# aws/sagemaker-xgboost-container

Measured on NVIDIA H100. Metric: boosting rounds/sec, higher is better.
Workload: dtype int64

## Files before the change

sagemaker-xgboost-container_b200/csrc/engine.h:

```cpp
#pragma once
#include <cuda_runtime.h>
#include <cstdint>
#include <cstdio>
#include <stdexcept>
#include <string>
#include <vector>

namespace b200 {

struct Error : std::runtime_error { using std::runtime_error::runtime_error; };
#define B200_CHECK(cond, msg) do { if (!(cond)) throw ::b200::Error(std::string(msg)); } while (0)
#define CUDA_OK(expr) do { cudaError_t e_ = (expr); if (e_ != cudaSuccess) throw ::b200::Error( \
    std::string("CUDA error: ") + cudaGetErrorString(e_) + " at " + __FILE__ + ":" + std::to_string(__LINE__)); } while (0)

extern long long g_kernel_launches;

cudaStream_t engine_stream();
int engine_num_sms();

template <typename T> struct DevBuf {
  T* p = nullptr; size_t n = 0;
  DevBuf() = default;
  DevBuf(const DevBuf&) = delete; DevBuf& operator=(const DevBuf&) = delete;
  ~DevBuf() { release(); }
// ... 46 lines not shown
inline int objective_transform(int o) {
  if (o == kBinaryLogistic || o == kRegLogistic) return kTransformSigmoid;
  if (objective_is_log_link(o)) return kTransformExp;
  return o == kHinge ? kTransformHinge : kTransformNone;
}

struct TrainParam {
  int objective = kSquaredError;
  int num_class = 1;
  int max_depth = 6, max_leaves = 0, max_bin = 256;
  int lossguide = 0;
  float eta = 0.3f, lambda = 1.0f, alpha = 0.0f, gamma = 0.0f, min_child_weight = 1.0f, max_delta_step = 0.0f;
  float scale_pos_weight = 1.0f, subsample = 1.0f, colsample_bytree = 1.0f, colsample_bylevel = 1.0f, colsample_bynode = 1.0f;
  unsigned seed = 0;
  int num_parallel_tree = 1;
  float huber_slope = 1.0f, tweedie_variance_power = 1.5f, poisson_max_delta_step = 0.7f;
};

struct SplitCand {
  float loss_chg; int feature; int bin; int dleft; int ord;
  long long GL, HL;
};

struct TreeArrays {
  int *left, *right, *parent, *split_index, *split_bin;
  unsigned char* default_left;
  float *split_cond, *base_weight, *loss_chg, *sum_hess;
};

struct GrowState {
  unsigned* seg_begin; unsigned* seg_count;
  int* hist_slot;
  GH64* node_sum;
  float* root_gain; float* weight;
  SplitCand* best;
  SplitCand* best_group;
  int* level_nodes;
  int* level_count;
  int* build_nid; int* build_sub_nid; int* build_parent_slot; int* build_count;
  unsigned* build_prefix;
  int* part_action;
  unsigned* tile_prefix;
  unsigned long long* tile_desc;
  unsigned* part_ctl;
  int* n_nodes; int* n_leaves;
  int* depth; unsigned char* open; int* n_slots; int* lg_done;
  float* lower; float* upper;
  float* scales;
  unsigned* absmax;
};

}
```

sagemaker-xgboost-container_b200/csrc/grow.cu:

```cuda
#include "grow.h"
#include <algorithm>
#include <cmath>
#include <cstdlib>
#include <cstring>
#include "comm.h"

namespace b200 {

__global__ void pack_tree_kernel(TreeArrays t, const int* n_nodes, DevNode* out, int cap) {
  const int nn = *n_nodes;
  for (int i = blockIdx.x * blockDim.x + threadIdx.x; i < cap; i += gridDim.x * blockDim.x) {
    DevNode d;
    if (i < nn) { d.cond = t.split_cond[i]; d.left = t.left[i]; d.right = t.right[i]; d.fidx_dl = (unsigned)t.split_index[i] | ((unsigned)t.default_left[i] << 31); }
    else { d.cond = 0.f; d.left = -1; d.right = -1; d.fidx_dl = 0; }
    out[i] = d;
  }
}
__global__ void snapshot_h_kernel(const GH64* slot, long long* cache, size_t entries) {
  for (size_t e = (size_t)blockIdx.x * blockDim.x + threadIdx.x; e < entries; e += (size_t)gridDim.x * blockDim.x) cache[e] = slot[e].h;
}
__global__ void slot_from_cache_kernel(GH64* slot, const long long* cache, size_t entries) {
  for (size_t e = (size_t)blockIdx.x * blockDim.x + threadIdx.x; e < entries; e += (size_t)gridDim.x * blockDim.x) { GH64 v; v.g = 0; v.h = cache[e]; slot[e] = v; }
}
__global__ void gather_u32_kernel(const unsigned* src, const unsigned* idx, unsigned* dst, int64_t n) {
  const int64_t i = (int64_t)blockIdx.x * blockDim.x + threadIdx.x;
  if (i < n) dst[i] = src[idx[i]];
}

void* PinnedPool::take(size_t bytes) {
  bytes = (bytes + 255) & ~(size_t)255;
  while (cur < chunks.size() && off + bytes > chunks[cur].second) { ++cur; off = 0; }
  if (cur >= chunks.size()) { size_t sz = std::max<size_t>(bytes, 4u << 20); char* p = nullptr; CUDA_OK(cudaMallocHost(&p, sz)); chunks.emplace_back(p, sz); off = 0; }
  void* r = chunks[cur].first + off; off += bytes; return r;
}
static bool tail_by_position(const BinnedMatrix& bm) { return bm.tw == 4 && !bm.tail_in_gather; }

size_t TreeBuilder::carve(GrowState& gs, uintptr_t base) const {
  const size_t N = cap_nodes, L = max_level_nodes, nblocks = ngroups + (tw > 0 ? 1 : 0);
  size_t off = 0;
  auto take = [&](auto*& p, size_t bytes) { p = reinterpret_cast<std::remove_reference_t<decltype(p)>>(base + off); off += (bytes + 255) & ~(size_t)255; };
  take(gs.seg_begin, 4 * N); take(gs.seg_count, 4 * N); take(gs.hist_slot, 4 * N); take(gs.node_sum, 16 * N); take(gs.root_gain, 4 * N); take(gs.weight, 4 * N);
  take(gs.best, sizeof(SplitCand) * N); take(gs.best_group, sizeof(SplitCand) * N * nblocks);
  take(gs.level_nodes, 4 * (size_t)(kMaxDepth + 1) * L); take(gs.level_count, 4 * (kMaxDepth + 2));
  take(gs.build_nid, 4 * L); take(gs.build_sub_nid, 4 * L); take(gs.build_parent_slot, 4 * L); take(gs.build_count, 4); take(gs.build_prefix, 4 * (L + 1));
  take(gs.part_action, 4 * L); take(gs.tile_prefix, 4 * (L + 1));
  take(gs.tile_desc, 8 * ((size_t)max_tiles + 1)); gs.part_ctl = (unsigned*)(gs.tile_desc + max_tiles);
  take(gs.n_leaves, 4); take(gs.scales, 16); take(gs.absmax, 8);
  take(gs.depth, 4 * N); take(gs.open, N); take(gs.n_slots, 4); take(gs.lg_done, 4); take(gs.lower, 4 * N); take(gs.upper, 4 * N);
  return off;
}

void TreeBuilder::ensure(const BinnedMatrix& bm, int max_depth_, int K, int lg_iters_, int n_ic_) {
  const bool tail_pos_ = tail_by_position(bm);
  const int64_t stride_ = (bm.n + 63) & ~(int64_t)63;
  if (n == bm.n && F == bm.F && ngroups == bm.ngroups && tw == bm.tw && tail_pos == tail_pos_ && max_depth == max_depth_ && lg_iters == lg_iters_ &&
      n_ic == n_ic_ && gpair.n >= (size_t)stride_ * K + 512) return;
  if (lg_iters_ == 0) B200_CHECK(max_depth_ >= 1 && max_depth_ <= kMaxDepth, "max_depth must be in [1, 16] for the B200 depth-wise hist builder");
  n = bm.n; F = bm.F; ngroups = bm.ngroups; tw = bm.tw; tail_pos = tail_pos_; max_depth = max_depth_; lg_iters = lg_iters_; n_ic = n_ic_;
  gp_stride = stride_; root_h_valid = false;
  cudaStream_t s = engine_stream();
  if (peer_reduce_active()) {
    peer_reduce_close();
    DevBuf<unsigned> bar; bar.alloc(1); bar.zero(s);
    Comm::get().allreduce_max_u32(bar.p, 1, s);
    Comm::get().sync_stream(s);
  }
  for (auto& tg : graphs) tg.destroy();
  size_t pool_slots; int max_nodes;
// ... 3 lines not shown
  } else {
    max_nodes = (1 << (max_depth + 1)) - 1; max_level_nodes = 1 << (max_depth - 1); region = max_level_nodes;
    pool_slots = 2 * (size_t)region;
  }
  cap_nodes = (max_nodes + 15) & ~15;
  slot_stride = hist_slot_entries(ngroups, tw);
  const size_t pool_bytes = pool_slots * slot_stride * sizeof(GH64);
  size_t free_b = 0, total_b = 0; cudaMemGetInfo(&free_b, &total_b);
  B200_CHECK(pool_bytes < free_b / 2 + hist_pool.n * sizeof(GH64), "histogram pool for this max_depth / max_leaves / feature count does not fit in device memory");
  hist_pool.alloc(pool_slots * slot_stride);
  gpair.alloc((size_t)gp_stride * K + 512); gpair.zero(s); err.alloc(1); tree_index_dev.alloc(1);
  if (!leaf_scale.p) { leaf_scale.alloc(1); set_leaf_scale(1.0f); }
  root_h_cache.alloc(slot_stride);
  for (int i = 0; i < 2; ++i) { ridx[i].alloc(n); gp[i].alloc(n); tl[i].alloc(tail_pos ? n : 0); }
  max_tiles = (unsigned)((n + kPartTile - 1) / kPartTile) + max_level_nodes + 1;
  scratch.alloc(3 * (size_t)max_level_nodes + 8);
  state_block.alloc(carve(gs, 0)); state_block.zero(s);
  carve(gs, (uintptr_t)state_block.p);
  tree_block.alloc(tree_block_bytes(cap_nodes));
  const TreeBlock tb = tree_block_layout(tree_block.p, cap_nodes);
  gs.n_nodes = tb.n_nodes; ta = tb.t; packed.alloc(cap_nodes);
  ic_path.alloc(n_ic ? (size_t)cap_nodes * F : 0); ic_allowed.alloc(n_ic ? (size_t)cap_nodes * F : 0);
  ic_sets.alloc((size_t)n_ic * F); ic_sets_host.clear();
  hist_configure();
  global_n = n;
  if (Comm::get().distributed()) {
    peer_reduce_setup({{hist_pool.p, hist_pool.n * sizeof(GH64)}, {state_block.p, state_block.n}}, s);
    DevBuf<double> dsum; dsum.alloc(1); double v = (double)n;
    CUDA_OK(cudaMemcpyAsync(dsum.p, &v, sizeof v, cudaMemcpyHostToDevice, s));
    Comm::get().allreduce_sum_f64(dsum.p, 1, s);
    CUDA_OK(cudaMemcpyAsync(&v, dsum.p, sizeof v, cudaMemcpyDeviceToHost, s));
    Comm::get().sync_stream(s);
    global_n = (int64_t)v;
  }
}

void TreeBuilder::set_leaf_scale(float v) {
  cudaStream_t s = engine_stream();
  CUDA_OK(cudaMemcpyAsync(leaf_scale.p, &v, sizeof v, cudaMemcpyHostToDevice, s));
  Comm::get().sync_stream(s);
}

const unsigned char* TreeBuilder::upload_mask(const std::string& mask, int tree_index) {
  cudaStream_t s = engine_stream(); feat_mask.ensure(mask.size());
  CUDA_OK(cudaMemcpyAsync(feat_mask.p, mask.data(), mask.size(), cudaMemcpyHostToDevice, s));
  CUDA_OK(cudaMemcpyAsync(tree_index_dev.p, &tree_index, sizeof(int), cudaMemcpyHostToDevice, s));
  Comm::get().sync_stream(s); return feat_mask.p;
// ... 115 lines not shown
  for (int it = 0; it < in.lg_iters; ++it) {
    launch_apply_lossguide(apply_args(in, 0, 0, 0), it, s);
    const PartArgs pa = part_args(0, it == 0 ? kRootRows : 0, 1);
    timed(kProfPartition, [&] { launch_partition(pa, max_tiles, s); });
    launch_lg_copy_back(pa, ridx[0].p, gp[0].p, tl[0].p, max_tiles, s);
    launch_zero_build_slots(gs, hist_pool.p, slot_stride, 1, s);
    timed(kProfDeepHist, [&] { launch_hist_build(level_hist_args(0), num_sms, s); });
    if (dist) {
      launch_lg_stage(gs, hist_pool.p, slot_stride, 1, s);
      allreduce_hist(hist_pool.p + (size_t)kLgStageSlot * slot_stride, slot_stride * 2);
      launch_lg_stage(gs, hist_pool.p, slot_stride, 0, s);
    }
    launch_subtract(gs, hist_pool.p, slot_stride, 1, s);
    launch_eval(eval_args(in, 1, nullptr), 2, s);
  }
  for (int L = 0; L < D && in.lg_iters == 0; ++L) {
    const bool final_level = (L == D - 1);
    const int next_base = ((L + 1) & 1) * region, next_half = 1 << L;
    launch_apply(apply_args(in, L, next_base, next_half), s);
    if (final_level) break;
    PartArgs pa = part_args(L, L == 0 ? kRootRows : (L & 1) ^ 1, L & 1);
    pa.build_only = L == D - 2 ? 1 : 0;
    timed(kProfPartition, [&] { launch_partition(pa, max_tiles, s); });
    CUDA_OK(cudaMemsetAsync(hist_pool.p + (size_t)next_base * slot_stride, 0, (size_t)next_half * slot_stride * sizeof(GH64), s));
    timed(kProfDeepHist, [&] { launch_hist_build(level_hist_args(L & 1), num_sms, s); });
    allreduce_hist(hist_pool.p + (size_t)next_base * slot_stride, (size_t)next_half * slot_stride * 2);
    launch_subtract(gs, hist_pool.p, slot_stride, next_half, s);
    launch_eval(eval_args(in, L + 1, in.mask ? in.mask + (size_t)(L + 1) * bm.F : nullptr), 1 << (L + 1), s);
  }
  timed(kProfMargin, [&] { launch_update_margin(ta, gs.n_nodes, bm.bins_col, bm.n, bm.has_missing, in.margin, in.K, k, leaf_scale.p, s); });
  if (profile) prof_margin_rows += bm.n;
  pack_tree_kernel<<<(cap_nodes + 255) / 256, 256, 0, s>>>(ta, gs.n_nodes, packed.p, cap_nodes); ++g_kernel_launches;
  CUDA_OK(cudaGetLastError());
}
void TreeBuilder::end_segment() {
  cudaGraph_t graph = nullptr; cudaGraphExec_t exec = nullptr;
  CUDA_OK(cudaStreamEndCapture(engine_stream(), &graph));
  cudaError_t e = cudaGraphInstantiate(&exec, graph, 0);
  cudaGraphDestroy(graph);
  CUDA_OK(e);
  capturing->segs.push_back(exec);
}

void TreeBuilder::grow(const TreeInputs& in) {
  cudaStream_t s = engine_stream();
  static const bool no_graph = getenv("B200XGB_NO_GRAPH") != nullptr;
  if ((int)graphs.size() <= in.k) graphs.resize(in.k + 1);
// ... 159 lines not shown
```

sagemaker-xgboost-container_b200/csrc/tree.cu:

```cuda
#include <type_traits>
#include "engine.h"
#include "rng.h"
#include "tree.h"

namespace b200 {

__device__ __forceinline__ double threshold_l1(double w, double alpha) {
  if (w > +alpha) return w - alpha;
  if (w < -alpha) return w + alpha;
  return 0.0;
}
__device__ __forceinline__ float calc_weight(const TrainParamDev& p, double G, double H) {
  if (H < p.min_child_weight || H <= 0.0) return 0.0f;
  double dw = -threshold_l1(G, p.alpha) / (H + p.lambda);
  if (p.max_delta_step != 0.0f && fabs(dw) > p.max_delta_step) dw = copysign((double)p.max_delta_step, dw);
  return (float)dw;
}
__device__ __forceinline__ float gain_at_weight_f(float g, float h, float lambda, float w) {
  return -__fadd_rn(__fmul_rn(__fmul_rn(2.0f, g), w), __fmul_rn(__fmul_rn(__fadd_rn(h, lambda), w), w));
}
__device__ __forceinline__ float calc_gain_given_weight(const TrainParamDev& p, double G, double H, float w) {
  if (H <= 0.0) return 0.0f;
  if (p.max_delta_step == 0.0f) { double t = threshold_l1(G, p.alpha); return (float)(t * t / (H + p.lambda)); }
  return gain_at_weight_f((float)G, (float)H, p.lambda, w);
// ... 239 lines not shown
  const int cb = a.cut_ptrs[best.feature];
  const float thr = best.dleft ? (best.bin < 0 ? a.min_vals[best.feature] : a.cut_vals[cb + best.bin]) : a.cut_vals[cb + best.bin];
  t.left[nid] = Lc; t.right[nid] = Rc; t.split_index[nid] = best.feature; t.split_cond[nid] = thr;
  t.split_bin[nid] = best.bin; t.default_left[nid] = (unsigned char)best.dleft;
  t.base_weight[nid] = gs.weight[nid]; t.loss_chg[nid] = best.loss_chg; t.sum_hess[nid] = (float)((double)tot.h * ish);
  const int ch[2] = {Lc, Rc}; const float cw[2] = {wl, wr}; const double chh[2] = {HL, HR};
  for (int s = 0; s < 2; ++s) {
    const int c = ch[s];
    t.left[c] = -1; t.right[c] = -1; t.parent[c] = nid; t.split_index[c] = 0; t.split_bin[c] = -1; t.default_left[c] = 0;
    t.split_cond[c] = a.p.eta * cw[s]; t.base_weight[c] = a.p.eta * cw[s]; t.loss_chg[c] = 0.f; t.sum_hess[c] = (float)chh[s];
  }
  gs.node_sum[Lc].g = GLq; gs.node_sum[Lc].h = HLq; gs.node_sum[Rc].g = GRq; gs.node_sum[Rc].h = HRq;
  gs.seg_begin[Lc] = 0; gs.seg_count[Lc] = 0; gs.seg_begin[Rc] = 0; gs.seg_count[Rc] = 0;
}

__device__ __forceinline__ void plan_child_hists(const GrowState& gs, int r, int nid, const SplitCand& best, const GH64& tot, int Lc, int Rc,
                                                 int bld_slot, int sub_slot) {
  const bool fewer_right = tot.h - best.HL < best.HL;
  const int bld = fewer_right ? Rc : Lc, sub = fewer_right ? Lc : Rc;
  gs.hist_slot[bld] = bld_slot; gs.hist_slot[sub] = sub_slot;
  gs.build_nid[r] = bld; gs.build_sub_nid[r] = sub; gs.build_parent_slot[r] = gs.hist_slot[nid];
}

__global__ void __launch_bounds__(256) apply_kernel(ApplyArgs a) {
  __shared__ unsigned s_tmp[33];
  GrowState& gs = a.gs;
  const int L = a.level;
  const int cnt = gs.level_count[L];
  const int* nodes = gs.level_nodes + (size_t)L * a.max_level_nodes;
  unsigned* valid = a.scratch;
  unsigned* rank = a.scratch + a.max_level_nodes;
  unsigned* tiles = a.scratch + 2 * (size_t)a.max_level_nodes;
  const double isg = (double)gs.scales[2], ish = (double)gs.scales[3];
  if (L == 0 && threadIdx.x == 0 && cnt > 0) finish_root(a, ish);
  for (int i = threadIdx.x; i < cnt; i += blockDim.x) {
    const int nid = nodes[i];
    const SplitCand best = best_of_blocks(a, nid);
    valid[i] = split_is_valid(a.p, best, gs.node_sum[nid], L) ? 1u : 0u;
  }
  __syncthreads();
  if (a.p.max_leaves > 0 && threadIdx.x == 0) {
    int leaves = *gs.n_leaves;
    for (int i = 0; i < cnt; ++i) { if (valid[i]) { if (leaves >= a.p.max_leaves) valid[i] = 0; else ++leaves; } }
  }
  __syncthreads();
  const unsigned nvalid = block_exclusive_scan(valid, rank, cnt, s_tmp);
  const int n0 = *gs.n_nodes;
  const bool children_evaluated = (L + 1 < a.p.max_depth) || a.p.max_depth == 0;
  for (int i = threadIdx.x; i < cnt; i += blockDim.x) {
    const int nid = nodes[i];
    tiles[i] = (gs.seg_count[nid] + kPartTile - 1) / kPartTile;
    gs.part_action[i] = (int)valid[i];
    if (!valid[i]) continue;
    const SplitCand best = gs.best[nid];
    const GH64 tot = gs.node_sum[nid];
    const int r = (int)rank[i];
    const int Lc = n0 + 2 * r, Rc = Lc + 1;
    expand_node(a, nid, best, tot, Lc, Rc, isg, ish);
    if (children_evaluated) {
      int* nxt = gs.level_nodes + (size_t)(L + 1) * a.max_level_nodes;
      nxt[2 * r] = Lc; nxt[2 * r + 1] = Rc;
      plan_child_hists(gs, r, nid, best, tot, Lc, Rc, a.next_base + r, a.next_base + a.next_half + r);
    }
  }
  __syncthreads();
  const unsigned total_tiles = block_exclusive_scan(tiles, gs.tile_prefix, cnt, s_tmp);
  if (threadIdx.x == 0) {
    gs.tile_prefix[cnt] = total_tiles;
    *gs.n_nodes = n0 + 2 * (int)nvalid;
    *gs.n_leaves += (int)nvalid;
    gs.level_count[L + 1] = children_evaluated ? 2 * (int)nvalid : 0;
    *gs.build_count = children_evaluated ? (int)nvalid : 0;
  }
}

__global__ void __launch_bounds__(256) apply_lossguide_kernel(ApplyArgs a, int iter) {
  __shared__ unsigned long long s_key[8];
  GrowState& gs = a.gs;
  const double isg = (double)gs.scales[2], ish = (double)gs.scales[3];
  const int src = iter == 0 ? 0 : 1;
  const int cnt = gs.level_count[src];
  const int* nodes = gs.level_nodes + (size_t)src * a.max_level_nodes;
  if (iter == 0 && threadIdx.x == 0 && cnt > 0) finish_root(a, ish);
  for (int i = threadIdx.x; i < cnt; i += blockDim.x) {
    const int nid = nodes[i];
    gs.open[nid] = best_of_blocks(a, nid).loss_chg > 1e-6f ? 1 : 0;
  }
  __syncthreads();
  const int n0 = *gs.n_nodes;
  unsigned long long key = 0ull;
  for (int nid = threadIdx.x; nid < n0; nid += blockDim.x)
    if (gs.open[nid]) { unsigned long long k = ((unsigned long long)__float_as_uint(gs.best[nid].loss_chg) << 32) | (unsigned long long)(0xffffffffu - (unsigned)nid); key = k > key ? k : key; }
#pragma unroll
  for (int o = 16; o > 0; o >>= 1) { unsigned long long x = __shfl_xor_sync(0xffffffffu, key, o); key = x > key ? x : key; }
  if ((threadIdx.x & 31) == 0) s_key[threadIdx.x >> 5] = key;
  __syncthreads();
  if (threadIdx.x != 0) return;
  for (int w = 1; w < 8; ++w) key = s_key[w] > key ? s_key[w] : key;
  bool stop = *gs.lg_done != 0 || key == 0ull;
  int nid = 0; SplitCand best{}; GH64 tot{};
  if (!stop) {
    nid = (int)(0xffffffffu - (unsigned)(key & 0xffffffffull));
    best = gs.best[nid]; tot = gs.node_sum[nid];
    stop = !split_is_valid(a.p, best, tot, gs.depth[nid]) || (a.p.max_leaves > 0 && *gs.n_leaves == a.p.max_leaves);
  }
  if (stop) {
    *gs.lg_done = 1;
    gs.level_count[0] = 0; gs.level_count[1] = 0; *gs.build_count = 0; gs.part_action[0] = 0; gs.tile_prefix[0] = 0; gs.tile_prefix[1] = 0;
    return;
  }
  gs.open[nid] = 0;
  const int Lc = n0, Rc = n0 + 1, d = gs.depth[nid];
  expand_node(a, nid, best, tot, Lc, Rc, isg, ish);
  gs.depth[Lc] = d + 1; gs.depth[Rc] = d + 1; gs.open[Lc] = 0; gs.open[Rc] = 0;
  *gs.n_nodes = n0 + 2;
  const int leaves = *gs.n_leaves + 1;
  *gs.n_leaves = leaves;
  const bool children_evaluated = !(a.p.max_depth > 0 && d + 1 >= a.p.max_depth) && !(a.p.max_leaves > 0 && leaves >= a.p.max_leaves);
  gs.level_nodes[0] = nid; gs.level_count[0] = 1;
  gs.part_action[0] = children_evaluated ? 1 : 0;
  gs.tile_prefix[0] = 0; gs.tile_prefix[1] = children_evaluated ? (gs.seg_count[nid] + kPartTile - 1) / kPartTile : 0u;
  if (children_evaluated) {
    int* nxt = gs.level_nodes + (size_t)a.max_level_nodes;
    nxt[0] = Lc; nxt[1] = Rc; gs.level_count[1] = 2;
    const int slot = (*gs.n_slots)++;
    plan_child_hists(gs, 0, nid, best, tot, Lc, Rc, slot, gs.hist_slot[nid]);
    *gs.build_count = 1;
  } else { gs.level_count[1] = 0; *gs.build_count = 0; }
}

template <typename Pay>
__global__ void __launch_bounds__(256) lg_copy_back_kernel(PartArgs a, unsigned* ridx_dst, Pay* gp_dst, unsigned* tl_dst) {
  const GrowState& gs = a.gs;
  if (gs.level_count[0] <= 0 || !gs.part_action[0]) return;
  const int nid = gs.level_nodes[0];
  const unsigned b = gs.seg_begin[nid], c = gs.seg_count[nid];
  const Pay* gp_src = static_cast<const Pay*>(a.gp_next);
  for (unsigned p = b + blockIdx.x * blockDim.x + threadIdx.x; p < b + c; p += gridDim.x * blockDim.x) {
    ridx_dst[p] = a.ridx_next[p]; gp_dst[p] = gp_src[p];
    if (a.tl_next) tl_dst[p] = a.tl_next[p];
  }
}

__global__ void __launch_bounds__(256) zero_build_slots_kernel(GrowState gs, GH64* pool, size_t stride) {
  const int r = blockIdx.x;
  if (r >= *gs.build_count) return;
  GH64* h = pool + (size_t)gs.hist_slot[gs.build_nid[r]] * stride;
  GH64 z; z.g = 0; z.h = 0;
  for (size_t e = (size_t)blockIdx.y * blockDim.x + threadIdx.x; e < stride; e += (size_t)gridDim.y * blockDim.x) h[e] = z;
}

__global__ void __launch_bounds__(256) lg_stage_kernel(GrowState gs, GH64* pool, size_t stride, int to_stage) {
  if (*gs.build_count <= 0) return;
  GH64* slot = pool + (size_t)gs.hist_slot[gs.build_nid[0]] * stride;
  GH64* stage = pool + (size_t)kLgStageSlot * stride;
  for (size_t e = (size_t)blockIdx.x * blockDim.x + threadIdx.x; e < stride; e += (size_t)gridDim.x * blockDim.x) {
    if (to_stage) stage[e] = slot[e]; else slot[e] = stage[e];
  }
}

__device__ __forceinline__ int find_node_of_tile(const unsigned* tile_prefix, int cnt, unsigned tile) {
  int lo = 0, hi = cnt;
  while (hi - lo > 1) { int mid = (lo + hi) >> 1; if (tile_prefix[mid] <= tile) lo = mid; else hi = mid; }
  return lo;
}

constexpr unsigned long long kDescAggregate = 1ull << 62;
constexpr unsigned long long kDescPrefix = 2ull << 62;

__device__ __forceinline__ unsigned long long ld_relaxed_u64(const unsigned long long* p) {
  unsigned long long v; asm volatile("ld.relaxed.gpu.global.u64 %0, [%1];" : "=l"(v) : "l"(p) : "memory"); return v;
}
__device__ __forceinline__ void st_relaxed_u64(unsigned long long* p, unsigned long long v) {
  asm volatile("st.relaxed.gpu.global.u64 [%0], %1;" :: "l"(p), "l"(v) : "memory");
}

__device__ unsigned lookback_lefts(const unsigned long long* d, unsigned lt) {
  const int lane = threadIdx.x & 31;
  unsigned acc = 0;
  for (int hi = (int)lt - 1; hi >= 0; hi -= 32) {
    const int j = hi - lane;
    unsigned long long v = 0;
    if (j >= 0) { v = ld_relaxed_u64(d + j); while ((v >> 62) == 0) { __nanosleep(64); v = ld_relaxed_u64(d + j); } }
    const unsigned pref = __ballot_sync(0xffffffffu, (v >> 62) == 2);
    const int last = pref ? __ffs(pref) - 1 : 31;
    unsigned x = lane <= last ? (unsigned)v : 0u;
#pragma unroll
    for (int o = 16; o > 0; o >>= 1) x += __shfl_xor_sync(0xffffffffu, x, o);
    acc += x;
    if (pref) break;
  }
  return acc;
}

template <bool GONLY, bool TL>
__global__ void __launch_bounds__(256, GONLY ? (TL ? 5 : 6) : 4) part_kernel(PartArgs a) {
  typedef typename std::conditional<GONLY, float, float2>::type Pay;
  GrowState& gs = a.gs;
  __shared__ unsigned s_rid[kPartTile];
  __shared__ Pay s_gp[kPartTile];
  __shared__ unsigned s_tl[TL ? kPartTile : 1];
  __shared__ unsigned s_w[8];
  const int cnt = gs.level_count[a.level];
  const unsigned total = cnt > 0 ? gs.tile_prefix[cnt] : 0u;
  if (threadIdx.x == 0) s_w[0] = atomicAdd(gs.part_ctl, 1u);
  __syncthreads();
  const unsigned tile = s_w[0];
  __syncthreads();
  const int i = tile < total ? find_node_of_tile(gs.tile_prefix, cnt, tile) : 0;
  if (tile < total && gs.part_action[i]) {
    const int nid = gs.level_nodes[(size_t)a.level * a.max_level_nodes + i];
    const unsigned t0 = gs.tile_prefix[i], lt = tile - t0;
    const unsigned b = gs.seg_begin[nid], c = gs.seg_count[nid];
    const unsigned p0 = b + lt * kPartTile, p1 = (b + c < p0 + kPartTile) ? b + c : p0 + kPartTile;
    const unsigned nrows = p1 - p0;
    const int f = a.tree.split_index[nid];
    const int sb = a.tree.split_bin[nid], dl = a.tree.default_left[nid];
    const uint8_t* col = a.bins_col + (int64_t)f * a.n;
    const Pay* gp_cur = static_cast<const Pay*>(a.gp_cur);
    Pay* gp_next = static_cast<Pay*>(a.gp_next);
    const unsigned pt = p0 + threadIdx.x * 8;
    unsigned rows[8]; Pay gp[8]; unsigned tl[8]; unsigned char fl[8]; unsigned mine = 0;
#pragma unroll
    for (int j = 0; j < 8; ++j) {
      const unsigned p = pt + j;
      rows[j] = 0; gp[j] = Pay{}; tl[j] = 0u;
      if (p < p1) {
        rows[j] = a.ridx_cur ? a.ridx_cur[p] : p;
        if constexpr (GONLY) gp[j] = static_cast<const float*>(a.gp_cur)[(size_t)p * a.gp_cur_stride];
        else gp[j] = gp_cur[p];
        if constexpr (TL) tl[j] = a.tl_cur[p];
      }
    }
#pragma unroll
    for (int j = 0; j < 8; ++j) {
      if (pt + j < p1) {
        const int byte = col[rows[j]];
        const bool left = (a.has_missing && byte == kMissingBin) ? (dl != 0) : (byte <= sb);
        fl[j] = left ? 1 : 0; mine += fl[j];
      } else fl[j] = 2;
    }
    const int lane = threadIdx.x & 31, warp = threadIdx.x >> 5;
    unsigned x = mine;
#pragma unroll
    for (int o = 1; o < 32; o <<= 1) { unsigned y = __shfl_up_sync(0xffffffffu, x, o); if (lane >= o) x += y; }
    if (lane == 31) s_w[warp] = x;
    __syncthreads();
    unsigned woff = 0, tile_left = 0;
    for (int w = 0; w < 8; ++w) { if (w < warp) woff += s_w[w]; tile_left += s_w[w]; }
    unsigned long long* desc = gs.tile_desc + t0;
    if (threadIdx.x == 0) st_relaxed_u64(desc + lt, (lt == 0 ? kDescPrefix : kDescAggregate) | tile_left);
    unsigned lbefore = woff + x - mine;
#pragma unroll
    for (int j = 0; j < 8; ++j) {
      if (fl[j] == 2) continue;
      const unsigned jj = threadIdx.x * 8 + j;
      const unsigned slot = fl[j] ? lbefore++ : tile_left + (jj - lbefore);
      s_rid[slot] = rows[j]; s_gp[slot] = gp[j]; if constexpr (TL) s_tl[slot] = tl[j];
    }
    unsigned lefts_before = 0;
    if (warp == 0 && lt > 0) {
      lefts_before = lookback_lefts(desc, lt);
      if (lane == 0) st_relaxed_u64(desc + lt, kDescPrefix | (lefts_before + tile_left));
    }
    __syncthreads();
    if (threadIdx.x == 0) s_w[0] = lefts_before;
    __syncthreads();
    lefts_before = s_w[0];
    const unsigned rights_before = lt * kPartTile - lefts_before;
    const int Lc = a.tree.left[nid], Rc = a.tree.right[nid];
    bool write_left = true, write_right = true;
    if (a.build_only) { const bool build_right = gs.node_sum[Rc].h < gs.node_sum[Lc].h; write_left = !build_right; write_right = build_right; }
    const unsigned k0 = write_left ? 0u : tile_left, k1 = write_right ? nrows : tile_left;
    const unsigned dl0 = b + lefts_before, dr0 = b + c - 1 - rights_before + tile_left;
    for (unsigned k = k0 + threadIdx.x; k < k1; k += blockDim.x) {
      const unsigned dest = k < tile_left ? dl0 + k : dr0 - k;
      a.ridx_next[dest] = s_rid[k];
      gp_next[dest] = s_gp[k];
      if constexpr (TL) a.tl_next[dest] = s_tl[k];
    }
    if (threadIdx.x == 0) {
      if (lt == gs.tile_prefix[i + 1] - t0 - 1) {
        const unsigned nl = lefts_before + tile_left;
        gs.seg_begin[Lc] = b; gs.seg_count[Lc] = nl; gs.seg_begin[Rc] = b + nl; gs.seg_count[Rc] = c - nl;
      }
      if (a.rows_counter) { atomicAdd(a.rows_counter, (unsigned long long)nrows); atomicAdd(a.rows_counter + 1, (unsigned long long)(k1 - k0)); }
    }
  }
  __syncthreads();
  if (threadIdx.x == 0) { __threadfence(); s_w[0] = atomicAdd(gs.part_ctl + 1, 1u) == gridDim.x - 1 ? 1u : 0u; }
  __syncthreads();
  if (!s_w[0]) return;
  __threadfence();
  const int nb = *gs.build_count;
  for (int r = threadIdx.x; r < nb; r += blockDim.x) gs.build_prefix[r] = __ldcg(gs.seg_count + gs.build_nid[r]);
  __syncthreads();
  const unsigned tot = nb > 0 ? block_exclusive_scan(gs.build_prefix, gs.build_prefix, nb, s_rid ) : 0u;
  if (threadIdx.x == 0) gs.build_prefix[nb > 0 ? nb : 0] = tot;
}

struct PackedNode { unsigned feat; unsigned short bin_dl; unsigned short left; };
constexpr int kPackedNodesSmem = 2048;
static_assert(sizeof(PackedNode) == 8, "PackedNode is 8 B");

__global__ void __launch_bounds__(256) update_margin_kernel(TreeArrays t, const int* n_nodes, const uint8_t* bins_col, int64_t n, int has_missing,
                                                            float* margin, int K, int k, const float* leaf_scale) {
  __shared__ PackedNode s_nodes[kPackedNodesSmem];
  __shared__ float s_leaf[kPackedNodesSmem];
  const int nn = *n_nodes;
  const bool packed = nn <= kPackedNodesSmem && nn < 0xffff;
  if (packed) {
    for (int i = threadIdx.x; i < nn; i += blockDim.x) {
      PackedNode p; p.feat = (unsigned)t.split_index[i]; p.bin_dl = (unsigned short)((t.split_bin[i] + 1) | (t.default_left[i] ? 0x8000 : 0));
      const int l = t.left[i]; p.left = l < 0 ? 0xffff : (unsigned short)l;
      s_nodes[i] = p; s_leaf[i] = t.split_cond[i];
    }
    __syncthreads();
  }
  const int64_t base = (int64_t)blockIdx.x * 1024 + threadIdx.x;
  int nid[4]; bool done[4];
  const bool root_leaf = packed ? (s_nodes[0].left == 0xffff) : (t.left[0] == -1);
// ... 39 lines not shown
  GH64* hs = pool + (size_t)gs.hist_slot[sub] * stride;
  for (size_t e = (size_t)blockIdx.y * blockDim.x + threadIdx.x; e < stride; e += (size_t)gridDim.y * blockDim.x) {
    GH64 p = hp[e], b = hb[e]; GH64 o; o.g = p.g - b.g; o.h = p.h - b.h; hs[e] = o;
  }
}

void launch_init_tree(const GrowState& gs, const TreeArrays& t, unsigned n, cudaStream_t s) {
  init_tree_kernel<<<1, 32, 0, s>>>(gs, t, n); ++g_kernel_launches; CUDA_OK(cudaGetLastError());
}
void launch_scales(const GrowState& gs, int grad_bits, cudaStream_t s) { scales_kernel<<<1, 32, 0, s>>>(gs, grad_bits); ++g_kernel_launches; CUDA_OK(cudaGetLastError()); }
void launch_eval(const EvalArgs& a, int max_nodes_level, cudaStream_t s) {
  dim3 grid(max_nodes_level, a.ngroups + (a.tw > 0 ? 1 : 0)); eval_kernel<<<grid, 32 * kEvalSegs, 0, s>>>(a); ++g_kernel_launches; CUDA_OK(cudaGetLastError());
}
void launch_apply_lossguide(const ApplyArgs& a, int iter, cudaStream_t s) { apply_lossguide_kernel<<<1, 256, 0, s>>>(a, iter); ++g_kernel_launches; CUDA_OK(cudaGetLastError()); }
void launch_lg_copy_back(const PartArgs& a, unsigned* ridx_dst, void* gp_dst, unsigned* tl_dst, unsigned max_tiles, cudaStream_t s) {
  const unsigned grid = max_tiles < 1184u ? max_tiles : 1184u;
  if (a.g_only) lg_copy_back_kernel<float><<<grid, 256, 0, s>>>(a, ridx_dst, static_cast<float*>(gp_dst), tl_dst);
  else lg_copy_back_kernel<float2><<<grid, 256, 0, s>>>(a, ridx_dst, static_cast<float2*>(gp_dst), tl_dst);
  ++g_kernel_launches; CUDA_OK(cudaGetLastError());
}
void launch_zero_build_slots(const GrowState& gs, GH64* pool, size_t slot_entries, int max_build, cudaStream_t s) {
  dim3 grid(max_build, (unsigned)((slot_entries + 1023) / 1024)); zero_build_slots_kernel<<<grid, 256, 0, s>>>(gs, pool, slot_entries); ++g_kernel_launches; CUDA_OK(cudaGetLastError());
}
void launch_lg_stage(const GrowState& gs, GH64* pool, size_t slot_entries, int to_stage, cudaStream_t s) {
  lg_stage_kernel<<<(unsigned)((slot_entries + 1023) / 1024), 256, 0, s>>>(gs, pool, slot_entries, to_stage); ++g_kernel_launches; CUDA_OK(cudaGetLastError());
}
void launch_apply(const ApplyArgs& a, cudaStream_t s) { apply_kernel<<<1, 256, 0, s>>>(a); ++g_kernel_launches; CUDA_OK(cudaGetLastError()); }
void launch_partition(const PartArgs& a, unsigned max_tiles, cudaStream_t s) {
  CUDA_OK(cudaMemsetAsync(a.gs.tile_desc, 0, sizeof(unsigned long long) * ((size_t)max_tiles + 1), s));
  const bool tl = a.tl_cur != nullptr;
  if (a.g_only) { if (tl) part_kernel<true, true><<<max_tiles, 256, 0, s>>>(a); else part_kernel<true, false><<<max_tiles, 256, 0, s>>>(a); }
  else { if (tl) part_kernel<false, true><<<max_tiles, 256, 0, s>>>(a); else part_kernel<false, false><<<max_tiles, 256, 0, s>>>(a); }
  ++g_kernel_launches; CUDA_OK(cudaGetLastError());
}
void launch_update_margin(const TreeArrays& t, const int* n_nodes, const uint8_t* bins_col, int64_t n, int has_missing, float* margin, int K, int k,
                          const float* leaf_scale, cudaStream_t s) {
  if (n == 0) return;
  update_margin_kernel<<<(unsigned)((n + 1023) / 1024), 256, 0, s>>>(t, n_nodes, bins_col, n, has_missing, margin, K, k, leaf_scale); ++g_kernel_launches; CUDA_OK(cudaGetLastError());
}
void launch_subtract(const GrowState& gs, GH64* pool, size_t slot_entries, int max_build, cudaStream_t s) {
  dim3 grid(max_build, (unsigned)((slot_entries + 1023) / 1024)); subtract_kernel<<<grid, 256, 0, s>>>(gs, pool, slot_entries); ++g_kernel_launches; CUDA_OK(cudaGetLastError());
}

}
```

sagemaker-xgboost-container_b200/csrc/tree.h:

```cpp
#pragma once
#include "engine.h"

namespace b200 {

constexpr unsigned kPartTile = 2048;

struct TrainParamDev {
  float eta, lambda, alpha, gamma, min_child_weight, max_delta_step;
  int max_depth, max_leaves;
};

struct EvalArgs {
  const GH64* hist_pool; GrowState gs; const int* cut_ptrs; const unsigned char* feat_mask;
  TrainParamDev p; int F, ngroups, tw, ntail, has_missing, level, max_level_nodes;
  const int* monotone;
  const unsigned char* node_allowed;
  float colsample_bynode; unsigned seed; const int* tree_index;
};

struct ApplyArgs {
  GrowState gs; TreeArrays tree; const int* cut_ptrs; const float* cut_vals; const float* min_vals;
  TrainParamDev p; unsigned* scratch; int nblocks , level, max_level_nodes, next_base, next_half;
  const int* monotone;
  unsigned char* node_path; unsigned char* node_allowed; const unsigned char* ic_sets; int n_ic_sets, F;
// ... 22 lines not shown
  const float* gpos;
  const unsigned* ridx;
  const int* build_count;
  const int* build_nid;
  const unsigned* build_prefix;
  const unsigned* seg_begin;
  const int* hist_slot;
  const float* scales;
  GH64* hist_pool;
  GH64* node_sum;
  int ngroups;
  int ng_chunk;
  int accumulate_sum;
  int g_only;
  int window_rows;
  int force_gather;
  unsigned long long* rows_counter;
};

constexpr int kLgRootSlot = 0, kLgStageSlot = 1, kLgFirstFreeSlot = 2;
void launch_apply_lossguide(const ApplyArgs& a, int iter, cudaStream_t s);
void launch_lg_copy_back(const PartArgs& a, unsigned* ridx_dst, void* gp_dst, unsigned* tl_dst, unsigned max_tiles, cudaStream_t s);
void launch_zero_build_slots(const GrowState& gs, GH64* pool, size_t slot_entries, int max_build, cudaStream_t s);
void launch_lg_stage(const GrowState& gs, GH64* pool, size_t slot_entries, int to_stage, cudaStream_t s);
void launch_hist_build(const HistArgs& a, int num_sms, cudaStream_t stream);
void hist_configure();
const char* hist_last_kernel();
void launch_init_tree(const GrowState& gs, const TreeArrays& t, unsigned n, cudaStream_t s);
void launch_scales(const GrowState& gs, int grad_bits, cudaStream_t s);
void launch_eval(const EvalArgs& a, int max_nodes_level, cudaStream_t s);
void launch_apply(const ApplyArgs& a, cudaStream_t s);
void launch_partition(const PartArgs& a, unsigned max_tiles, cudaStream_t s);
void launch_update_margin(const TreeArrays& t, const int* n_nodes, const uint8_t* bins_col, int64_t n, int has_missing, float* margin, int K, int k,
                          const float* leaf_scale, cudaStream_t s);
void launch_subtract(const GrowState& gs, GH64* pool, size_t slot_entries, int max_build, cudaStream_t s);

}
```

Measured before the change: 74.99.

## Restructure partition kernel with precomputed node plans, cp.async payload staging, ballot compaction

Apply kernels now write a compact PartNode record (segment, tile offset, split feature/bin, children, flags) so each partition CTA loads one struct instead of chasing several tree arrays. Warp 0 finds the tile's node with a ballot search. Gradient and tail payloads are staged through cp.async into shared memory, and the compaction uses warp ballots with a source-index indirection. The last-block build_prefix scan is moved into new zero-slot kernels, which replace a memset. Occupancy bounds and the shared-memory carveout are raised, at the cost of added register and shared-memory pressure and more synchronization complexity.

Measured after the change: 76.82 (median of 6 runs). +2.4%, better.

```diff
diff --git a/sagemaker-xgboost-container_b200/csrc/engine.h b/sagemaker-xgboost-container_b200/csrc/engine.h
--- a/sagemaker-xgboost-container_b200/csrc/engine.h
+++ b/sagemaker-xgboost-container_b200/csrc/engine.h
@@ -92,6 +92,14 @@
   long long GL, HL;
 };
 
+struct PartNode {
+  unsigned seg_begin, seg_count;
+  unsigned tile0;
+  int feature, split_bin;
+  int left, right;
+  unsigned flags;
+};
+
 struct TreeArrays {
   int *left, *right, *parent, *split_index, *split_bin;
   unsigned char* default_left;
@@ -110,6 +118,7 @@
   int* build_nid; int* build_sub_nid; int* build_parent_slot; int* build_count;
   unsigned* build_prefix;
   int* part_action;
+  PartNode* part_node;
   unsigned* tile_prefix;
   unsigned long long* tile_desc;
   unsigned* part_ctl;
diff --git a/sagemaker-xgboost-container_b200/csrc/grow.cu b/sagemaker-xgboost-container_b200/csrc/grow.cu
--- a/sagemaker-xgboost-container_b200/csrc/grow.cu
+++ b/sagemaker-xgboost-container_b200/csrc/grow.cu
@@ -43,7 +43,7 @@
   take(gs.best, sizeof(SplitCand) * N); take(gs.best_group, sizeof(SplitCand) * N * nblocks);
   take(gs.level_nodes, 4 * (size_t)(kMaxDepth + 1) * L); take(gs.level_count, 4 * (kMaxDepth + 2));
   take(gs.build_nid, 4 * L); take(gs.build_sub_nid, 4 * L); take(gs.build_parent_slot, 4 * L); take(gs.build_count, 4); take(gs.build_prefix, 4 * (L + 1));
-  take(gs.part_action, 4 * L); take(gs.tile_prefix, 4 * (L + 1));
+  take(gs.part_action, 4 * L); take(gs.part_node, sizeof(PartNode) * L); take(gs.tile_prefix, 4 * (L + 1));
   take(gs.tile_desc, 8 * ((size_t)max_tiles + 1)); gs.part_ctl = (unsigned*)(gs.tile_desc + max_tiles);
   take(gs.n_leaves, 4); take(gs.scales, 16); take(gs.absmax, 8);
   take(gs.depth, 4 * N); take(gs.open, N); take(gs.n_slots, 4); take(gs.lg_done, 4); take(gs.lower, 4 * N); take(gs.upper, 4 * N);
@@ -93,7 +93,7 @@
   gs.n_nodes = tb.n_nodes; ta = tb.t; packed.alloc(cap_nodes);
   ic_path.alloc(n_ic ? (size_t)cap_nodes * F : 0); ic_allowed.alloc(n_ic ? (size_t)cap_nodes * F : 0);
   ic_sets.alloc((size_t)n_ic * F); ic_sets_host.clear();
-  hist_configure();
+  hist_configure(); part_configure();
   global_n = n;
   if (Comm::get().distributed()) {
     peer_reduce_setup({{hist_pool.p, hist_pool.n * sizeof(GH64)}, {state_block.p, state_block.n}}, s);
@@ -255,7 +255,7 @@
     PartArgs pa = part_args(L, L == 0 ? kRootRows : (L & 1) ^ 1, L & 1);
     pa.build_only = L == D - 2 ? 1 : 0;
     timed(kProfPartition, [&] { launch_partition(pa, max_tiles, s); });
-    CUDA_OK(cudaMemsetAsync(hist_pool.p + (size_t)next_base * slot_stride, 0, (size_t)next_half * slot_stride * sizeof(GH64), s));
+    launch_zero_level_slots(gs, hist_pool.p + (size_t)next_base * slot_stride, (size_t)next_half * slot_stride, s);
     timed(kProfDeepHist, [&] { launch_hist_build(level_hist_args(L & 1), num_sms, s); });
     allreduce_hist(hist_pool.p + (size_t)next_base * slot_stride, (size_t)next_half * slot_stride * 2);
     launch_subtract(gs, hist_pool.p, slot_stride, next_half, s);
diff --git a/sagemaker-xgboost-container_b200/csrc/tree.cu b/sagemaker-xgboost-container_b200/csrc/tree.cu
--- a/sagemaker-xgboost-container_b200/csrc/tree.cu
+++ b/sagemaker-xgboost-container_b200/csrc/tree.cu
@@ -1,3 +1,4 @@
+#include <algorithm>
 #include <type_traits>
 #include "engine.h"
 #include "rng.h"
@@ -285,6 +286,14 @@
   gs.build_nid[r] = bld; gs.build_sub_nid[r] = sub; gs.build_parent_slot[r] = gs.hist_slot[nid];
 }
 
+__device__ __forceinline__ void plan_partition(const GrowState& gs, int i, int nid, const SplitCand& best, const GH64& tot, int Lc, int Rc, unsigned tile0) {
+  PartNode pn;
+  pn.seg_begin = gs.seg_begin[nid]; pn.seg_count = gs.seg_count[nid]; pn.tile0 = tile0;
+  pn.feature = best.feature; pn.split_bin = best.bin; pn.left = Lc; pn.right = Rc;
+  pn.flags = (best.dleft ? 1u : 0u) | (tot.h - best.HL < best.HL ? 2u : 0u);
+  gs.part_node[i] = pn;
+}
+
 __global__ void __launch_bounds__(256) apply_kernel(ApplyArgs a) {
   __shared__ unsigned s_tmp[33];
   GrowState& gs = a.gs;
@@ -308,17 +317,20 @@
   }
   __syncthreads();
   const unsigned nvalid = block_exclusive_scan(valid, rank, cnt, s_tmp);
+  for (int i = threadIdx.x; i < cnt; i += blockDim.x) tiles[i] = valid[i] ? (gs.seg_count[nodes[i]] + kPartTile - 1) / kPartTile : 0u;
+  __syncthreads();
+  const unsigned total_tiles = block_exclusive_scan(tiles, gs.tile_prefix, cnt, s_tmp);
   const int n0 = *gs.n_nodes;
   const bool children_evaluated = (L + 1 < a.p.max_depth) || a.p.max_depth == 0;
   for (int i = threadIdx.x; i < cnt; i += blockDim.x) {
     const int nid = nodes[i];
-    tiles[i] = (gs.seg_count[nid] + kPartTile - 1) / kPartTile;
     gs.part_action[i] = (int)valid[i];
     if (!valid[i]) continue;
     const SplitCand best = gs.best[nid];
     const GH64 tot = gs.node_sum[nid];
     const int r = (int)rank[i];
     const int Lc = n0 + 2 * r, Rc = Lc + 1;
+    plan_partition(gs, i, nid, best, tot, Lc, Rc, gs.tile_prefix[i]);
     expand_node(a, nid, best, tot, Lc, Rc, isg, ish);
     if (children_evaluated) {
       int* nxt = gs.level_nodes + (size_t)(L + 1) * a.max_level_nodes;
@@ -327,7 +339,6 @@
     }
   }
   __syncthreads();
-  const unsigned total_tiles = block_exclusive_scan(tiles, gs.tile_prefix, cnt, s_tmp);
   if (threadIdx.x == 0) {
     gs.tile_prefix[cnt] = total_tiles;
     *gs.n_nodes = n0 + 2 * (int)nvalid;
@@ -374,6 +385,7 @@
   }
   gs.open[nid] = 0;
   const int Lc = n0, Rc = n0 + 1, d = gs.depth[nid];
+  plan_partition(gs, 0, nid, best, tot, Lc, Rc, 0u);
   expand_node(a, nid, best, tot, Lc, Rc, isg, ish);
   gs.depth[Lc] = d + 1; gs.depth[Rc] = d + 1; gs.open[Lc] = 0; gs.open[Rc] = 0;
   *gs.n_nodes = n0 + 2;
@@ -405,7 +417,24 @@
   }
 }
 
+__device__ void write_build_prefix(const GrowState& gs, unsigned* s_tmp ) {
+  const int nb = *gs.build_count;
+  for (int r = threadIdx.x; r < nb; r += blockDim.x) gs.build_prefix[r] = gs.seg_count[gs.build_nid[r]];
+  __syncthreads();
+  const unsigned tot = nb > 0 ? block_exclusive_scan(gs.build_prefix, gs.build_prefix, nb, s_tmp) : 0u;
+  if (threadIdx.x == 0) gs.build_prefix[nb > 0 ? nb : 0] = tot;
+}
+
+__global__ void __launch_bounds__(256) zero_level_slots_kernel(GrowState gs, GH64* slots, size_t entries) {
+  __shared__ unsigned s_tmp[33];
+  if (blockIdx.x == 0) write_build_prefix(gs, s_tmp);
+  GH64 z; z.g = 0; z.h = 0;
+  for (size_t e = (size_t)blockIdx.x * blockDim.x + threadIdx.x; e < entries; e += (size_t)gridDim.x * blockDim.x) slots[e] = z;
+}
+
 __global__ void __launch_bounds__(256) zero_build_slots_kernel(GrowState gs, GH64* pool, size_t stride) {
+  __shared__ unsigned s_tmp[33];
+  if (blockIdx.x == 0 && blockIdx.y == 0) write_build_prefix(gs, s_tmp);
   const int r = blockIdx.x;
   if (r >= *gs.build_count) return;
   GH64* h = pool + (size_t)gs.hist_slot[gs.build_nid[r]] * stride;
@@ -422,10 +451,19 @@
   }
 }
 
-__device__ __forceinline__ int find_node_of_tile(const unsigned* tile_prefix, int cnt, unsigned tile) {
-  int lo = 0, hi = cnt;
-  while (hi - lo > 1) { int mid = (lo + hi) >> 1; if (tile_prefix[mid] <= tile) lo = mid; else hi = mid; }
-  return lo;
+__device__ __forceinline__ int find_node_of_tile(const unsigned* tile_prefix, const int* level_count, unsigned tile) {
+  const int lane = threadIdx.x & 31;
+  const unsigned v0 = tile_prefix[lane];
+  const int cnt = *level_count;
+  int i = 0;
+  for (int base = 0; base <= cnt; base += 32) {
+    const int j = base + lane;
+    const unsigned v = base == 0 ? v0 : (j <= cnt ? tile_prefix[j] : 0xffffffffu);
+    const unsigned m = __ballot_sync(0xffffffffu, j <= cnt && v <= tile);
+    if (m) i = base + 31 - __clz(m);
+    if (m != 0xffffffffu) break;
+  }
+  return i < cnt ? i : -1;
 }
 
 constexpr unsigned long long kDescAggregate = 1ull << 62;
@@ -456,110 +494,122 @@
   return acc;
 }
 
+template <int B> __device__ __forceinline__ void cp_async(void* smem, const void* gmem) {
+  const unsigned s = (unsigned)__cvta_generic_to_shared(smem);
+  asm volatile("cp.async.ca.shared.global [%0], [%1], %2;" :: "r"(s), "l"(gmem), "n"(B) : "memory");
+}
+__device__ __forceinline__ void cp_async_wait_all() { asm volatile("cp.async.wait_all;" ::: "memory"); }
+
+template <bool GONLY, bool TL> constexpr int part_ctas_per_sm() { return GONLY ? (TL ? 7 : 8) : (TL ? 5 : 6); }
 template <bool GONLY, bool TL>
-__global__ void __launch_bounds__(256, GONLY ? (TL ? 5 : 6) : 4) part_kernel(PartArgs a) {
+__global__ void __launch_bounds__(256, part_ctas_per_sm<GONLY, TL>()) part_kernel(PartArgs a) {
   typedef typename std::conditional<GONLY, float, float2>::type Pay;
   GrowState& gs = a.gs;
   __shared__ unsigned s_rid[kPartTile];
+  __shared__ unsigned short s_src[kPartTile];
   __shared__ Pay s_gp[kPartTile];
   __shared__ unsigned s_tl[TL ? kPartTile : 1];
   __shared__ unsigned s_w[8];
-  const int cnt = gs.level_count[a.level];
-  const unsigned total = cnt > 0 ? gs.tile_prefix[cnt] : 0u;
-  if (threadIdx.x == 0) s_w[0] = atomicAdd(gs.part_ctl, 1u);
-  __syncthreads();
-  const unsigned tile = s_w[0];
-  __syncthreads();
-  const int i = tile < total ? find_node_of_tile(gs.tile_prefix, cnt, tile) : 0;
-  if (tile < total && gs.part_action[i]) {
-    const int nid = gs.level_nodes[(size_t)a.level * a.max_level_nodes + i];
-    const unsigned t0 = gs.tile_prefix[i], lt = tile - t0;
-    const unsigned b = gs.seg_begin[nid], c = gs.seg_count[nid];
-    const unsigned p0 = b + lt * kPartTile, p1 = (b + c < p0 + kPartTile) ? b + c : p0 + kPartTile;
-    const unsigned nrows = p1 - p0;
-    const int f = a.tree.split_index[nid];
-    const int sb = a.tree.split_bin[nid], dl = a.tree.default_left[nid];
-    const uint8_t* col = a.bins_col + (int64_t)f * a.n;
-    const Pay* gp_cur = static_cast<const Pay*>(a.gp_cur);
-    Pay* gp_next = static_cast<Pay*>(a.gp_next);
-    const unsigned pt = p0 + threadIdx.x * 8;
-    unsigned rows[8]; Pay gp[8]; unsigned tl[8]; unsigned char fl[8]; unsigned mine = 0;
-#pragma unroll
-    for (int j = 0; j < 8; ++j) {
-      const unsigned p = pt + j;
-      rows[j] = 0; gp[j] = Pay{}; tl[j] = 0u;
-      if (p < p1) {
-        rows[j] = a.ridx_cur ? a.ridx_cur[p] : p;
-        if constexpr (GONLY) gp[j] = static_cast<const float*>(a.gp_cur)[(size_t)p * a.gp_cur_stride];
-        else gp[j] = gp_cur[p];
-        if constexpr (TL) tl[j] = a.tl_cur[p];
-      }
-    }
-#pragma unroll
-    for (int j = 0; j < 8; ++j) {
-      if (pt + j < p1) {
-        const int byte = col[rows[j]];
-        const bool left = (a.has_missing && byte == kMissingBin) ? (dl != 0) : (byte <= sb);
-        fl[j] = left ? 1 : 0; mine += fl[j];
-      } else fl[j] = 2;
-    }
-    const int lane = threadIdx.x & 31, warp = threadIdx.x >> 5;
-    unsigned x = mine;
-#pragma unroll
-    for (int o = 1; o < 32; o <<= 1) { unsigned y = __shfl_up_sync(0xffffffffu, x, o); if (lane >= o) x += y; }
-    if (lane == 31) s_w[warp] = x;
-    __syncthreads();
-    unsigned woff = 0, tile_left = 0;
-    for (int w = 0; w < 8; ++w) { if (w < warp) woff += s_w[w]; tile_left += s_w[w]; }
-    unsigned long long* desc = gs.tile_desc + t0;
-    if (threadIdx.x == 0) st_relaxed_u64(desc + lt, (lt == 0 ? kDescPrefix : kDescAggregate) | tile_left);
-    unsigned lbefore = woff + x - mine;
-#pragma unroll
-    for (int j = 0; j < 8; ++j) {
-      if (fl[j] == 2) continue;
-      const unsigned jj = threadIdx.x * 8 + j;
-      const unsigned slot = fl[j] ? lbefore++ : tile_left + (jj - lbefore);
-      s_rid[slot] = rows[j]; s_gp[slot] = gp[j]; if constexpr (TL) s_tl[slot] = tl[j];
-    }
-    unsigned lefts_before = 0;
-    if (warp == 0 && lt > 0) {
-      lefts_before = lookback_lefts(desc, lt);
-      if (lane == 0) st_relaxed_u64(desc + lt, kDescPrefix | (lefts_before + tile_left));
-    }
-    __syncthreads();
-    if (threadIdx.x == 0) s_w[0] = lefts_before;
-    __syncthreads();
-    lefts_before = s_w[0];
-    const unsigned rights_before = lt * kPartTile - lefts_before;
-    const int Lc = a.tree.left[nid], Rc = a.tree.right[nid];
-    bool write_left = true, write_right = true;
-    if (a.build_only) { const bool build_right = gs.node_sum[Rc].h < gs.node_sum[Lc].h; write_left = !build_right; write_right = build_right; }
-    const unsigned k0 = write_left ? 0u : tile_left, k1 = write_right ? nrows : tile_left;
-    const unsigned dl0 = b + lefts_before, dr0 = b + c - 1 - rights_before + tile_left;
-    for (unsigned k = k0 + threadIdx.x; k < k1; k += blockDim.x) {
-      const unsigned dest = k < tile_left ? dl0 + k : dr0 - k;
-      a.ridx_next[dest] = s_rid[k];
-      gp_next[dest] = s_gp[k];
-      if constexpr (TL) a.tl_next[dest] = s_tl[k];
-    }
-    if (threadIdx.x == 0) {
-      if (lt == gs.tile_prefix[i + 1] - t0 - 1) {
-        const unsigned nl = lefts_before + tile_left;
-        gs.seg_begin[Lc] = b; gs.seg_count[Lc] = nl; gs.seg_begin[Rc] = b + nl; gs.seg_count[Rc] = c - nl;
-      }
-      if (a.rows_counter) { atomicAdd(a.rows_counter, (unsigned long long)nrows); atomicAdd(a.rows_counter + 1, (unsigned long long)(k1 - k0)); }
-    }
-  }
-  __syncthreads();
-  if (threadIdx.x == 0) { __threadfence(); s_w[0] = atomicAdd(gs.part_ctl + 1, 1u) == gridDim.x - 1 ? 1u : 0u; }
-  __syncthreads();
-  if (!s_w[0]) return;
-  __threadfence();
-  const int nb = *gs.build_count;
-  for (int r = threadIdx.x; r < nb; r += blockDim.x) gs.build_prefix[r] = __ldcg(gs.seg_count + gs.build_nid[r]);
-  __syncthreads();
-  const unsigned tot = nb > 0 ? block_exclusive_scan(gs.build_prefix, gs.build_prefix, nb, s_rid ) : 0u;
-  if (threadIdx.x == 0) gs.build_prefix[nb > 0 ? nb : 0] = tot;
+  __shared__ PartNode s_node;
+  __shared__ unsigned s_lt;
+  const int lane = threadIdx.x & 31, warp = threadIdx.x >> 5;
+  if (warp == 0) {
+    unsigned tile = 0;
+    if (lane == 0) tile = atomicAdd(gs.part_ctl, 1u);
+    tile = __shfl_sync(0xffffffffu, tile, 0);
+    const int i = find_node_of_tile(gs.tile_prefix, gs.level_count + a.level, tile);
+    unsigned w = 0;
+    if (i >= 0 && lane < 8) { w = reinterpret_cast<const unsigned*>(gs.part_node + i)[lane]; reinterpret_cast<unsigned*>(&s_node)[lane] = w; }
+    const unsigned t0 = __shfl_sync(0xffffffffu, w, 2);
+    if (lane == 0) s_lt = i >= 0 ? tile - t0 : ~0u;
+  }
+  __syncthreads();
+  const unsigned lt = s_lt;
+  if (lt == ~0u) return;
+  const unsigned p0 = s_node.seg_begin + lt * kPartTile, nrows = min(s_node.seg_begin + s_node.seg_count - p0, kPartTile);
+  const int sb = s_node.split_bin;
+  const int miss = a.has_missing ? kMissingBin : -1, miss_left = (s_node.flags & 1u) ? 1 : 0;
+  const uint8_t* col = a.bins_col + (int64_t)s_node.feature * a.n;
+  const Pay* gp_cur = static_cast<const Pay*>(a.gp_cur);
+  Pay* gp_next = static_cast<Pay*>(a.gp_next);
+  const unsigned q0 = (unsigned)warp * 256 + lane, pq = p0 + q0;
+  const unsigned* rid_in = a.ridx_cur ? a.ridx_cur + pq : nullptr;
+  const float* g_in = static_cast<const float*>(a.gp_cur) + (size_t)pq * a.gp_cur_stride;
+  const bool g2 = a.gp_cur_stride == 2;
+  unsigned rows[8]; unsigned left = 0;
+#pragma unroll
+  for (int j = 0; j < 8; ++j) {
+    rows[j] = 0;
+    const unsigned q = q0 + 32 * j;
+    if (q < nrows) {
+      rows[j] = rid_in ? rid_in[32 * j] : pq + 32 * j;
+      if constexpr (GONLY) cp_async<4>(s_gp + q, g2 ? g_in + 64 * j : g_in + 32 * j);
+      else cp_async<8>(s_gp + q, gp_cur + pq + 32 * j);
+      if constexpr (TL) cp_async<4>(s_tl + q, a.tl_cur + pq + 32 * j);
+    }
+  }
+#pragma unroll
+  for (int j = 0; j < 8; ++j) {
+    if (q0 + 32 * j < nrows) {
+      const int byte = col[rows[j]];
+      const bool l = byte == miss ? miss_left : (byte <= sb);
+      left |= (l ? 1u : 0u) << j;
+    }
+  }
+  unsigned wl = 0;
+#pragma unroll
+  for (int j = 0; j < 8; ++j) wl += __popc(__ballot_sync(0xffffffffu, (left >> j) & 1u));
+  if (lane == 0) s_w[warp] = wl;
+  __syncthreads();
+  unsigned woff = 0, tile_left = 0;
+  for (int w = 0; w < 8; ++w) { if (w < warp) woff += s_w[w]; tile_left += s_w[w]; }
+  unsigned long long* desc = gs.tile_desc + s_node.tile0;
+  if (threadIdx.x == 0) st_relaxed_u64(desc + lt, (lt == 0 ? kDescPrefix : kDescAggregate) | tile_left);
+  const unsigned below = (1u << lane) - 1u;
+  unsigned lb = woff;
+#pragma unroll
+  for (int j = 0; j < 8; ++j) {
+    const unsigned m = __ballot_sync(0xffffffffu, (left >> j) & 1u);
+    const unsigned q = q0 + 32 * j;
+    if (q < nrows) {
+      const unsigned lq = lb + __popc(m & below);
+      const unsigned slot = ((left >> j) & 1u) ? lq : tile_left + (q - lq);
+      s_rid[slot] = rows[j]; s_src[slot] = (unsigned short)q;
+    }
+    lb += __popc(m);
+  }
+  unsigned lefts_before = 0;
+  if (warp == 0 && lt > 0) {
+    lefts_before = lookback_lefts(desc, lt);
+    if (lane == 0) st_relaxed_u64(desc + lt, kDescPrefix | (lefts_before + tile_left));
+  }
+  cp_async_wait_all();
+  __syncthreads();
+  if (threadIdx.x == 0) s_w[0] = lefts_before;
+  __syncthreads();
+  lefts_before = s_w[0];
+  const unsigned rights_before = lt * kPartTile - lefts_before;
+  const volatile PartNode& nv = s_node;
+  const unsigned b = nv.seg_begin, c = nv.seg_count;
+  bool write_left = true, write_right = true;
+  if (a.build_only) { const bool build_right = (s_node.flags & 2u) != 0; write_left = !build_right; write_right = build_right; }
+  const unsigned k0 = write_left ? 0u : tile_left, k1 = write_right ? nrows : tile_left;
+  const unsigned dl0 = b + lefts_before, dr0 = b + c - 1 - rights_before + tile_left;
+  for (unsigned k = k0 + threadIdx.x; k < k1; k += blockDim.x) {
+    const unsigned dest = k < tile_left ? dl0 + k : dr0 - k;
+    const unsigned q = s_src[k];
+    a.ridx_next[dest] = s_rid[k];
+    gp_next[dest] = s_gp[q];
+    if constexpr (TL) a.tl_next[dest] = s_tl[q];
+  }
+  if (threadIdx.x == 0) {
+    if (p0 + nrows == b + c) {
+      const unsigned nl = lefts_before + tile_left;
+      const int Lc = s_node.left, Rc = s_node.right;
+      gs.seg_begin[Lc] = b; gs.seg_count[Lc] = nl; gs.seg_begin[Rc] = b + nl; gs.seg_count[Rc] = c - nl;
+    }
+    if (a.rows_counter) { atomicAdd(a.rows_counter, (unsigned long long)nrows); atomicAdd(a.rows_counter + 1, (unsigned long long)(k1 - k0)); }
+  }
 }
 
 struct PackedNode { unsigned feat; unsigned short bin_dl; unsigned short left; };
@@ -645,10 +695,24 @@
 void launch_zero_build_slots(const GrowState& gs, GH64* pool, size_t slot_entries, int max_build, cudaStream_t s) {
   dim3 grid(max_build, (unsigned)((slot_entries + 1023) / 1024)); zero_build_slots_kernel<<<grid, 256, 0, s>>>(gs, pool, slot_entries); ++g_kernel_launches; CUDA_OK(cudaGetLastError());
 }
+void launch_zero_level_slots(const GrowState& gs, GH64* slots, size_t entries, cudaStream_t s) {
+  const size_t blocks = std::min<size_t>((entries + 1023) / 1024, (size_t)engine_num_sms() * 8);
+  zero_level_slots_kernel<<<(unsigned)std::max<size_t>(blocks, 1), 256, 0, s>>>(gs, slots, entries); ++g_kernel_launches; CUDA_OK(cudaGetLastError());
+}
 void launch_lg_stage(const GrowState& gs, GH64* pool, size_t slot_entries, int to_stage, cudaStream_t s) {
   lg_stage_kernel<<<(unsigned)((slot_entries + 1023) / 1024), 256, 0, s>>>(gs, pool, slot_entries, to_stage); ++g_kernel_launches; CUDA_OK(cudaGetLastError());
 }
 void launch_apply(const ApplyArgs& a, cudaStream_t s) { apply_kernel<<<1, 256, 0, s>>>(a); ++g_kernel_launches; CUDA_OK(cudaGetLastError()); }
+void part_configure() {
+  static bool done = false;
+  if (done) return;
+  const int c = (int)cudaSharedmemCarveoutMaxShared;
+  CUDA_OK(cudaFuncSetAttribute(part_kernel<true, true>, cudaFuncAttributePreferredSharedMemoryCarveout, c));
+  CUDA_OK(cudaFuncSetAttribute(part_kernel<true, false>, cudaFuncAttributePreferredSharedMemoryCarveout, c));
+  CUDA_OK(cudaFuncSetAttribute(part_kernel<false, true>, cudaFuncAttributePreferredSharedMemoryCarveout, c));
+  CUDA_OK(cudaFuncSetAttribute(part_kernel<false, false>, cudaFuncAttributePreferredSharedMemoryCarveout, c));
+  done = true;
+}
 void launch_partition(const PartArgs& a, unsigned max_tiles, cudaStream_t s) {
   CUDA_OK(cudaMemsetAsync(a.gs.tile_desc, 0, sizeof(unsigned long long) * ((size_t)max_tiles + 1), s));
   const bool tl = a.tl_cur != nullptr;
diff --git a/sagemaker-xgboost-container_b200/csrc/tree.h b/sagemaker-xgboost-container_b200/csrc/tree.h
--- a/sagemaker-xgboost-container_b200/csrc/tree.h
+++ b/sagemaker-xgboost-container_b200/csrc/tree.h
@@ -68,6 +68,7 @@
 void launch_apply_lossguide(const ApplyArgs& a, int iter, cudaStream_t s);
 void launch_lg_copy_back(const PartArgs& a, unsigned* ridx_dst, void* gp_dst, unsigned* tl_dst, unsigned max_tiles, cudaStream_t s);
 void launch_zero_build_slots(const GrowState& gs, GH64* pool, size_t slot_entries, int max_build, cudaStream_t s);
+void launch_zero_level_slots(const GrowState& gs, GH64* slots, size_t entries, cudaStream_t s);
 void launch_lg_stage(const GrowState& gs, GH64* pool, size_t slot_entries, int to_stage, cudaStream_t s);
 void launch_hist_build(const HistArgs& a, int num_sms, cudaStream_t stream);
 void hist_configure();
@@ -77,6 +78,7 @@
 void launch_eval(const EvalArgs& a, int max_nodes_level, cudaStream_t s);
 void launch_apply(const ApplyArgs& a, cudaStream_t s);
 void launch_partition(const PartArgs& a, unsigned max_tiles, cudaStream_t s);
+void part_configure();
 void launch_update_margin(const TreeArrays& t, const int* n_nodes, const uint8_t* bins_col, int64_t n, int has_missing, float* margin, int K, int k,
                           const float* leaf_scale, cudaStream_t s);
 void launch_subtract(const GrowState& gs, GH64* pool, size_t slot_entries, int max_build, cudaStream_t s);
```
